# mohakbhardwaj/mjmpc

Hardware: AMD Instinct MI355X
Metric: particle-steps/sec (reacher_7dof-v0 MPPI 4096p x H32 per GPU, control loop incl. noise, rollout, update, shift) (higher is better)
Workload: dtype f64

## Files before the change

### mjmpc_amd/csrc/arm_rollout.hip

```cpp
#include <hip/hip_runtime.h>

#include <cstdlib>
#include <type_traits>

#include "arm_model.h"
#include "arm_rollout.h"
#include "lanegroup.h"
#include "noise_device.h"

namespace mjmpc {
namespace {

template <typename T>
constexpr int newton_maxit() { return sizeof(T) == 4 ? 32 : 12; }

#define PHASE() asm volatile("" ::: "memory")
#define LDS_WAVE_SYNC()                                        \
    do {                                                       \
        __builtin_amdgcn_fence(__ATOMIC_ACQ_REL, "wavefront"); \
        asm volatile("" ::: "memory");                         \
        __builtin_amdgcn_sched_barrier(0);                     \
    } while (0)

constexpr int N_LINK_FIELDS = O_NV / LANES;
__device__ __forceinline__ float uniform_(float x) { return __int_as_float(__builtin_amdgcn_readfirstlane(__float_as_int(x))); }
__device__ __forceinline__ double uniform_(double x) {
    return __hiloint2double(__builtin_amdgcn_readfirstlane(__double2hiint(x)), __builtin_amdgcn_readfirstlane(__double2loint(x)));
}
#ifdef MJMPC_ARM_XJ
constexpr bool XJ = true;
#else
constexpr bool XJ = false;
#endif
template <typename T, bool REG>
struct Model {
    static constexpr bool cached = REG;
    const T* m;
    int l8;
    T reg[REG ? N_LINK_FIELDS : 1];
    T inv_width, mid, inv_mid, inv_omid, dmin, ddiff, solB, solK;
    int ipower;
    __device__ __forceinline__ void cache() {
        if constexpr (REG) {
#pragma unroll
            for (int k = 0; k < N_LINK_FIELDS; ++k) reg[k] = m[k * LANES + l8];
            mid = uniform_(m[O_SOL_MID]);
            inv_width = uniform_(rcp_(m[O_SOL_WIDTH]));
            inv_mid = uniform_(rcp_(mid));
            inv_omid = uniform_(rcp_(T(1) - mid));
            dmin = uniform_(m[O_SOL_DMIN]);
            ddiff = uniform_(m[O_SOL_DMAX] - m[O_SOL_DMIN]);
            solB = uniform_(m[O_SOL_B]);
            solK = uniform_(m[O_SOL_K]);
            ipower = __builtin_amdgcn_readfirstlane((int)m[O_SOL_POWER]);
        }
        cache_xj();
    }
    __device__ __forceinline__ T link(int off, int c = 0) const {
        if constexpr (REG) return reg[off / LANES + c];
        else return m[off + c * LANES + l8];
    }
    __device__ __forceinline__ T glob(int off, int c = 0) const { return m[off + c]; }
    bool xs = false;
    T xf = T(0), xD = T(0), xB = T(0);
    __device__ __forceinline__ void cache_xj() {
        if constexpr (XJ && REG) {
            xs = m[O_JTYPE + l8] != T(0);
            xf = m[O_FLOSS + l8];
            xD = m[O_FLOSS_D + l8];
            xB = uniform_(m[O_FLOSS_B]);
        }
    }
    __device__ __forceinline__ bool xj_slide() const { if constexpr (XJ && REG) return xs; else return XJ && m[O_JTYPE + l8] != T(0); }
    __device__ __forceinline__ T xj_floss() const { if constexpr (XJ && REG) return xf; else return m[O_FLOSS + l8]; }
    __device__ __forceinline__ T xj_floss_D() const { if constexpr (XJ && REG) return xD; else return m[O_FLOSS_D + l8]; }
    __device__ __forceinline__ T xj_floss_B() const { if constexpr (XJ && REG) return xB; else return m[O_FLOSS_B]; }
};

__device__ __forceinline__ float mul_rn(float a, float b) { return __fmul_rn(a, b); }
__device__ __forceinline__ double mul_rn(double a, double b) { return __dmul_rn(a, b); }
__device__ __forceinline__ float add_rn(float a, float b) { return __fadd_rn(a, b); }
__device__ __forceinline__ double add_rn(double a, double b) { return __dadd_rn(a, b); }

template <typename T>
__device__ __forceinline__ void cross(const T* a, const T* b, T* c) {
    c[0] = a[1] * b[2] - a[2] * b[1];
    c[1] = a[2] * b[0] - a[0] * b[2];
    c[2] = a[0] * b[1] - a[1] * b[0];
}
template <typename T>
__device__ __forceinline__ T dot(const T* a, const T* b) { return a[0] * b[0] + a[1] * b[1] + a[2] * b[2]; }
template <typename T>
__device__ __forceinline__ void matvec(const T* R, const T* x, T* y) {
    for (int i = 0; i < 3; ++i) y[i] = R[3 * i] * x[0] + R[3 * i + 1] * x[1] + R[3 * i + 2] * x[2];
}
template <typename T>
__device__ __forceinline__ void symvec(const T* S, const T* x, T* y) {
    y[0] = S[0] * x[0] + S[3] * x[1] + S[4] * x[2];
    y[1] = S[3] * x[0] + S[1] * x[1] + S[5] * x[2];
    y[2] = S[4] * x[0] + S[5] * x[1] + S[2] * x[2];
}

template <int S, typename T>
__device__ __forceinline__ void fk_scan_step(T* R, T* p, int l8) {
    T Ra[9], pa[3], Rn[9], t[3];
    for (int k = 0; k < 9; ++k) Ra[k] = (k % 4 == 0) ? shr<S>(R[k], T(1), l8) : shr0<S>(R[k], l8);
    for (int k = 0; k < 3; ++k) pa[k] = shr0<S>(p[k], l8);
    for (int i = 0; i < 3; ++i)
        for (int j = 0; j < 3; ++j)
            Rn[3 * i + j] = Ra[3 * i] * R[j] + Ra[3 * i + 1] * R[3 + j] + Ra[3 * i + 2] * R[6 + j];
    matvec(Ra, p, t);
    for (int k = 0; k < 3; ++k) p[k] = pa[k] + t[k];
    for (int k = 0; k < 9; ++k) R[k] = Rn[k];
}

template <typename T, typename MT>
__device__ __forceinline__ void row_params(const MT& M, T r, T diag_approx, T jv, T& D, T& aref) {
    if constexpr (MT::cached) {
        T x = fabs(r) * M.inv_width, y;
        x = x > T(1) ? T(1) : x;
        if (M.ipower == 2) {
            T om = T(1) - x;
            y = x <= M.mid ? x * x * M.inv_mid : T(1) - om * om * M.inv_omid;
        } else if (M.ipower == 1) {
            y = x;
        } else {
            const bool lo = x <= M.mid;
            const T xa = lo ? x : T(1) - x, ia = lo ? M.inv_mid : M.inv_omid;
            T qq = xa;
            for (int k = 1; k < M.ipower; ++k) qq *= xa * ia;
            y = lo ? qq : T(1) - qq;
        }
        const T imp = M.dmin + y * M.ddiff;
        T Rr = (T(1) - imp) * rcp_(imp) * diag_approx;
        Rr = Rr < T(1e-15) ? T(1e-15) : Rr;
        D = rcp_(Rr);
        aref = -M.solB * jv - M.solK * imp * r;
        return;
    }
    const T dmin = M.glob(O_SOL_DMIN), dmax = M.glob(O_SOL_DMAX), width = M.glob(O_SOL_WIDTH);
    const T mid = M.glob(O_SOL_MID), power = M.glob(O_SOL_POWER);
    T x = fabs(r) * rcp_(width), y;
    x = x > T(1) ? T(1) : x;
    if (power == T(2)) {
        T om = T(1) - x;
        y = x <= mid ? x * x * rcp_(mid) : T(1) - om * om * rcp_(T(1) - mid);
    } else if (power == T(1)) {
        y = x;
    } else {
        const int n = (int)power;
        const bool lo = x <= mid;
        const T xa = lo ? x : T(1) - x, ma = lo ? mid : T(1) - mid;
        T num = xa, den = T(1);
        for (int k = 1; k < n; ++k) {
            num *= xa;
            den *= ma;
        }
        const T qq = num * rcp_(den);
        y = lo ? qq : T(1) - qq;
    }
    T imp = dmin + y * (dmax - dmin);
    T Rr = (T(1) - imp) * rcp_(imp) * diag_approx;
    Rr = Rr < T(1e-15) ? T(1e-15) : Rr;
    D = rcp_(Rr);
    aref = -M.glob(O_SOL_B) * jv - M.glob(O_SOL_K) * imp * r;
}

template <typename T>
struct Dense {
    T a[21];
    T d[MAX_LINKS];
    static __device__ __forceinline__ constexpr int ix(int i, int j) { return i * (i - 1) / 2 + j; }

    __device__ __forceinline__ void load(const T* tile, const T* diag) {
#pragma unroll
        for (int i = 1; i < MAX_LINKS; ++i)
#pragma unroll
            for (int j = 0; j < i; ++j) a[ix(i, j)] = tile[i * LANES + j];
#pragma unroll
        for (int i = 0; i < MAX_LINKS; ++i) d[i] = diag[i];
    }
    __device__ __forceinline__ void add_rank1(T w, const T* jc) {
#pragma unroll
        for (int i = 0; i < MAX_LINKS; ++i) {
            const T wi = w * jc[i];
            d[i] += wi * jc[i];
#pragma unroll
            for (int j = 0; j < i; ++j) a[ix(i, j)] += wi * jc[j];
        }
    }
    __device__ __forceinline__ void factor() {
#pragma unroll
        for (int k = 0; k < MAX_LINKS; ++k) {
            const T inv = rcp_fast(d[k]);
            d[k] = inv;
#pragma unroll
            for (int i = k + 1; i < MAX_LINKS; ++i) {
                const T aik = a[ix(i, k)];
                const T lik = aik * inv;
#pragma unroll
                for (int j = k + 1; j < i; ++j) a[ix(i, j)] -= aik * a[ix(j, k)];
                d[i] -= aik * lik;
                a[ix(i, k)] = lik;
            }
        }
    }
    __device__ __forceinline__ void solve(T* b) const {
#pragma unroll
        for (int i = 1; i < MAX_LINKS; ++i)
#pragma unroll
            for (int j = 0; j < i; ++j) b[i] -= a[ix(i, j)] * b[j];
#pragma unroll
        for (int i = 0; i < MAX_LINKS; ++i) b[i] *= d[i];
#pragma unroll
        for (int i = MAX_LINKS - 2; i >= 0; --i)
#pragma unroll
            for (int j = i + 1; j < MAX_LINKS; ++j) b[i] -= a[ix(j, i)] * b[j];
    }
};

constexpr int V_DH = LANES * LANES, V_RH = V_DH + LANES, V_DE = V_RH + LANES, V_RE = V_DE + LANES, V_XH = V_RE + LANES,
              V_XE = V_XH + LANES, V_JC = V_XE + LANES, V_TAU = V_JC + LANES, V_EI = V_TAU + LANES,
              PSTRIDE = V_EI + LANES * LANES + 4,
              V_LS = V_XH, V_LD = V_DH, V_LA = V_RH;

template <int K, typename T>
__device__ __forceinline__ void cl_accumulate(const double* __restrict__ W, int A, int nv, int l8, T cq, T cv, double& u) {
    const double qk = (double)bcast<K>(cq), vk = (double)bcast<K>(cv);
    if (K < nv) u += W[K * A + l8] * qk + W[(nv + K) * A + l8] * vk;
    if constexpr (K + 1 < MAX_LINKS) cl_accumulate<K + 1, T>(W, A, nv, l8, cq, cv, u);
}

template <int S, typename T>
__device__ __forceinline__ void mass_diagonals(const T* sw, const T* sv, const T* Fn, const T* Ff, T* d) {
    if constexpr (S == 0) {
        d[0] = dot(sw, Fn) + dot(sv, Ff);
    } else {
        T fn[3], ff[3];
        for (int c = 0; c < 3; ++c) {
            fn[c] = shl_raw<S>(Fn[c]);
            ff[c] = shl_raw<S>(Ff[c]);
        }
        d[S] = dot(sw, fn) + dot(sv, ff);
    }
    if constexpr (S + 1 < MAX_LINKS) mass_diagonals<S + 1, T>(sw, sv, Fn, Ff, d);
}

struct ArmInts {
    int site_link, n_sphere, sph_link, frame_skip, nv;
};

template <typename T>
struct LinkFrame {
    T R[9], p[3], ax[3];
    T mass, a[3], cw[3];
    T Ib[6], hm[3];
    T sw[3], sv[3];
};

template <typename T, typename MT>
__device__ __forceinline__ void kinematics(const MT& M, T sq, T cq, int l8, LinkFrame<T>& L, T q = T(0)) {
    T* R = L.R;
    T* p = L.p;
    T* ax = L.ax;
    const T s = sq, c = cq, tt = T(1) - cq;
    for (int k = 0; k < 3; ++k) { ax[k] = M.link(O_AXIS, k); p[k] = M.link(O_OFF, k); }
    if constexpr (XJ) {
        const T qs = M.xj_slide() ? q : T(0);
        for (int k = 0; k < 3; ++k) p[k] += qs * ax[k];
    }
    R[0] = c + tt * ax[0] * ax[0];
    R[1] = tt * ax[0] * ax[1] - s * ax[2];
    R[2] = tt * ax[0] * ax[2] + s * ax[1];
    R[3] = tt * ax[0] * ax[1] + s * ax[2];
    R[4] = c + tt * ax[1] * ax[1];
    R[5] = tt * ax[1] * ax[2] - s * ax[0];
    R[6] = tt * ax[0] * ax[2] - s * ax[1];
    R[7] = tt * ax[1] * ax[2] + s * ax[0];
    R[8] = c + tt * ax[2] * ax[2];
    fk_scan_step<1>(R, p, l8);
    fk_scan_step<2>(R, p, l8);
    fk_scan_step<4>(R, p, l8);
}

template <typename T, typename MT>
__device__ __forceinline__ void link_frames(const MT& M, LinkFrame<T>& L) {
    const T* R = L.R;
    const T* p = L.p;
    const T mass = L.mass = M.link(O_MASS);
    T t3[3];
    matvec(R, L.ax, L.a);
    {
        const T com[3] = {M.link(O_COM, 0), M.link(O_COM, 1), M.link(O_COM, 2)};
        matvec(R, com, t3);
    }
    T* cw = L.cw;
    for (int k = 0; k < 3; ++k) cw[k] = p[k] + t3[k];
    T* Ib = L.Ib;
    {
        T Il[6], RI[9];
        for (int k = 0; k < 6; ++k) Il[k] = M.link(O_INERTIA, k);
        for (int i = 0; i < 3; ++i) {
            const T* r = R + 3 * i;
            RI[3 * i + 0] = r[0] * Il[0] + r[1] * Il[3] + r[2] * Il[4];
            RI[3 * i + 1] = r[0] * Il[3] + r[1] * Il[1] + r[2] * Il[5];
            RI[3 * i + 2] = r[0] * Il[4] + r[1] * Il[5] + r[2] * Il[2];
        }
        T cc = dot(cw, cw);
        Ib[0] = dot(RI + 0, R + 0) + mass * (cc - cw[0] * cw[0]);
        Ib[1] = dot(RI + 3, R + 3) + mass * (cc - cw[1] * cw[1]);
        Ib[2] = dot(RI + 6, R + 6) + mass * (cc - cw[2] * cw[2]);
        Ib[3] = dot(RI + 0, R + 3) - mass * cw[0] * cw[1];
        Ib[4] = dot(RI + 0, R + 6) - mass * cw[0] * cw[2];
        Ib[5] = dot(RI + 3, R + 6) - mass * cw[1] * cw[2];
    }
    for (int k = 0; k < 3; ++k) { L.hm[k] = mass * cw[k]; L.sw[k] = L.a[k]; }
    cross(p, L.a, L.sv);
    if constexpr (XJ) {
        if (M.xj_slide())
            for (int k = 0; k < 3; ++k) { L.sw[k] = T(0); L.sv[k] = L.a[k]; }
    }
}

template <typename T, typename MT>
__device__ __forceinline__ T bias_force(const MT& M, const LinkFrame<T>& L, T v, int l8) {
    const T *sw = L.sw, *sv = L.sv, *Ib = L.Ib, *hm = L.hm;
    const T mass = L.mass;
    T Vw[3], Vv[3];
    for (int k = 0; k < 3; ++k) {
        Vw[k] = psum(sw[k] * v, l8);
        Vv[k] = psum(sv[k] * v, l8);
    }
    T Aw[3], Av[3];
    {
        T xw[3] = {sw[0] * v, sw[1] * v, sw[2] * v}, xv[3] = {sv[0] * v, sv[1] * v, sv[2] * v};
        T dw[3], d1[3], d2[3];
        cross(Vw, xw, dw);
        cross(Vw, xv, d1);
        cross(Vv, xw, d2);
        for (int k = 0; k < 3; ++k) {
            Aw[k] = psum(dw[k], l8);
            Av[k] = psum(d1[k] + d2[k], l8) - M.glob(O_GRAVITY, k);
        }
    }
    T nV[3], fV[3], nA[3], fA[3], t1[3], t2[3];
    symvec(Ib, Vw, nV);
    cross(hm, Vv, t1);
    cross(hm, Vw, t2);
    for (int k = 0; k < 3; ++k) { nV[k] += t1[k]; fV[k] = mass * Vv[k] - t2[k]; }
    symvec(Ib, Aw, nA);
    cross(hm, Av, t1);
    cross(hm, Aw, t2);
    for (int k = 0; k < 3; ++k) { nA[k] += t1[k]; fA[k] = mass * Av[k] - t2[k]; }
    T c1[3], c2[3], c3[3];
    cross(Vw, nV, c1);
    cross(Vv, fV, c2);
    cross(Vw, fV, c3);
    T fn[3], ff[3];
    for (int k = 0; k < 3; ++k) {
        fn[k] = ssum(nA[k] + c1[k] + c2[k], l8);
        ff[k] = ssum(fA[k] + c3[k], l8);
    }
    return dot(sw, fn) + dot(sv, ff);
}

template <typename T>
__device__ __forceinline__ T mass_matrix_tile(const LinkFrame<T>& L, int l8, T* ldsM) {
    const T *sw = L.sw, *sv = L.sv;
    T d[MAX_LINKS];
    {
        T mc = ssum(L.mass, l8), hc[3], Ic[6];
        for (int k = 0; k < 3; ++k) hc[k] = ssum(L.hm[k], l8);
        for (int k = 0; k < 6; ++k) Ic[k] = ssum(L.Ib[k], l8);
        T Fn[3], Ff[3], t1[3], t2[3];
        symvec(Ic, sw, Fn);
        cross(hc, sv, t1);
        cross(hc, sw, t2);
        for (int k = 0; k < 3; ++k) { Fn[k] += t1[k]; Ff[k] = mc * sv[k] - t2[k]; }
        mass_diagonals<0, T>(sw, sv, Fn, Ff, d);
    }
#pragma unroll
    for (int sft = 0; sft < MAX_LINKS; ++sft) {
        if (l8 + sft < MAX_LINKS) {
            ldsM[l8 * LANES + l8 + sft] = d[sft];
            ldsM[(l8 + sft) * LANES + l8] = d[sft];
        }
    }
    return d[0];
}

template <int S0, int S1, typename T>
__device__ __forceinline__ T mass_matrix_tile_part(const LinkFrame<T>& L, int l8, T* ldsM) {
    const T *sw = L.sw, *sv = L.sv;
    T d[MAX_LINKS];
#pragma unroll
    for (int k = 0; k < MAX_LINKS; ++k) d[k] = T(0);
    T mc = ssum(L.mass, l8), hc[3], Ic[6];
    for (int k = 0; k < 3; ++k) hc[k] = ssum(L.hm[k], l8);
    for (int k = 0; k < 6; ++k) Ic[k] = ssum(L.Ib[k], l8);
    T Fn[3], Ff[3], t1[3], t2[3];
    symvec(Ic, sw, Fn);
    cross(hc, sv, t1);
    cross(hc, sw, t2);
    for (int k = 0; k < 3; ++k) { Fn[k] += t1[k]; Ff[k] = mc * sv[k] - t2[k]; }
    auto diag_s = [&](auto SC) {
        constexpr int S = decltype(SC)::value;
        if constexpr (S >= S0 && S < S1) {
            if constexpr (S == 0) {
                d[0] = dot(sw, Fn) + dot(sv, Ff);
            } else {
                T fn[3], ff[3];
                for (int c = 0; c < 3; ++c) { fn[c] = shl_raw<S>(Fn[c]); ff[c] = shl_raw<S>(Ff[c]); }
                d[S] = dot(sw, fn) + dot(sv, ff);
            }
        }
    };
    diag_s(std::integral_constant<int, 0>()); diag_s(std::integral_constant<int, 1>()); diag_s(std::integral_constant<int, 2>());
    diag_s(std::integral_constant<int, 3>()); diag_s(std::integral_constant<int, 4>()); diag_s(std::integral_constant<int, 5>());
    diag_s(std::integral_constant<int, 6>());
#pragma unroll
    for (int sft = S0; sft < S1; ++sft) {
        if (l8 + sft < MAX_LINKS) {
            ldsM[l8 * LANES + l8 + sft] = d[sft];
            ldsM[(l8 + sft) * LANES + l8] = d[sft];
        }
    }
    return d[0];
}

template <typename T, typename MT>
__device__ __forceinline__ void contact_geometry(const MT& M, const ArmInts& I, const LinkFrame<T>& L,
                                                 const T* ctr, T v, int l8, T& cdist, bool& cinst, T& jc, T& jv) {
    const T pn[3] = {M.glob(O_PLANE_N, 0), M.glob(O_PLANE_N, 1), M.glob(O_PLANE_N, 2)};
    const T sph_r = M.glob(O_SPH_R);
    cdist = dot(ctr, pn) - M.glob(O_PLANE_D) - sph_r;
    cinst = cdist < M.glob(O_SPH_MARGIN);
    jc = T(0);
    jv = T(0);
    if (__any(cinst)) {
        T r[3], ar[3];
        for (int k = 0; k < 3; ++k) r[k] = ctr[k] - pn[k] * (sph_r + T(0.5) * cdist) - L.p[k];
        cross(L.a, r, ar);
        T jl = dot(pn, ar);
        if constexpr (XJ) jl = M.xj_slide() ? dot(pn, L.a) : jl;
        jc = (cinst && l8 <= I.sph_link) ? jl : T(0);
        jv = gsum(jc * v);
    }
}

enum Role : int { SOLO = 0, DYN = 1, SOLVE = 2,
                  QDYN = 3, QSOLVE = 4, QMASS = 5, QAUX = 6 };
template <int ROLE>
__device__ __forceinline__ constexpr int role_slot() {
    return (ROLE == SOLVE || ROLE == QSOLVE) ? 1 : (ROLE == QMASS ? 2 : (ROLE == QAUX ? 3 : 0));
}
template <int ROLE>
__device__ __forceinline__ constexpr bool role_counts() { return ROLE == SOLO || ROLE == DYN || ROLE == QDYN; }

struct Stamps {
#if defined(MJMPC_STAMPS) && defined(MJMPC_STAMPS_ABS)
    long long acc[16];
    int nsub;
    __device__ __forceinline__ void begin() { for (int k = 0; k < 16; ++k) acc[k] = 0; nsub = 0; }
    __device__ __forceinline__ void mark(int k) {
        if (nsub == MJMPC_STAMPS_ABS) acc[k] = clock64();
        if (k == 13 || k == 15) ++nsub;
    }
    __device__ __forceinline__ void flush(unsigned* diag, int wave, int lane) {
        if (diag && blockIdx.x == 0 && lane == 0)
            for (int k = 0; k < 16; ++k) ((unsigned long long*)diag)[2 + 16 * wave + k] = (unsigned long long)acc[k];
    }
#elif defined(MJMPC_STAMPS)
    long long last, acc[16];
    __device__ __forceinline__ void begin() { for (int k = 0; k < 16; ++k) acc[k] = 0; last = clock64(); }
#ifdef MJMPC_STAMPS_MASK
    __device__ __forceinline__ void mark(int k) {
        if (!((MJMPC_STAMPS_MASK >> k) & 1)) return;
        const long long t = clock64(); acc[k] += t - last; last = t;
    }
#else
#ifdef MJMPC_STAMPS_FENCE
    __device__ __forceinline__ void mark(int k) {
        __builtin_amdgcn_sched_barrier(0);
        const long long t = clock64(); acc[k] += t - last; last = t;
        __builtin_amdgcn_sched_barrier(0);
    }
#else
    __device__ __forceinline__ void mark(int k) { const long long t = clock64(); acc[k] += t - last; last = t; }
#endif
#endif
    __device__ __forceinline__ void flush(unsigned* diag, int wave, int lane) {
        if (diag && blockIdx.x == 0 && lane == 0)
            for (int k = 0; k < 16; ++k) ((unsigned long long*)diag)[2 + 16 * wave + k] = (unsigned long long)acc[k];
    }
#else
    __device__ __forceinline__ void begin() {}
    __device__ __forceinline__ void mark(int) {}
    __device__ __forceinline__ void flush(unsigned*, int, int) {}
#endif
};

__device__ __forceinline__ void duo_barrier() {
    asm volatile("s_waitcnt lgkmcnt(0)\n\ts_barrier" ::: "memory");
    __builtin_amdgcn_sched_barrier(0);
}

template <typename T>
struct FlossRow {
    T f = T(0), D = T(0), aref = T(0);
    int z = 0;
    __device__ __forceinline__ int zone_at(T xa) const {
        if (!(f > T(0))) return 0;
        const T sl = D * (xa - aref);
        const T bc = sizeof(T) == 4 ? T(2e-5) * (fabs(sl) + f) : T(0);
        if (z < 0) return sl > -f + bc ? (sl >= f ? 1 : 0) : -1;
        if (z > 0) return sl < f - bc ? (sl <= -f ? -1 : 0) : 1;
        return sl <= -f - bc ? -1 : (sl >= f + bc ? 1 : 0);
    }
    __device__ __forceinline__ T diag() const { return (f > T(0) && z == 0) ? D : T(0); }
    __device__ __forceinline__ T rhs() const { return f > T(0) ? (z == 0 ? D * aref : (z < 0 ? f : -f)) : T(0); }
    __device__ __forceinline__ T force(T xa) const { return f > T(0) ? (z == 0 ? -D * (xa - aref) : (z < 0 ? f : -f)) : T(0); }
    __device__ __forceinline__ int memory() const { return f > T(0) ? (16 | ((z + 1) << 5)) : 0; }
};
template <typename T, typename MT>
__device__ __forceinline__ FlossRow<T> floss_row(const MT& M, T v, int rows) {
    FlossRow<T> r;
    if constexpr (XJ) {
        r.f = M.xj_floss();
        if (r.f > T(0)) {
            r.D = M.xj_floss_D();
            r.aref = -M.xj_floss_B() * v;
            r.z = (rows & 16) ? ((rows >> 5) & 3) - 1 : 0;
        }
    }
    return r;
}

template <typename T, typename MT>
__device__ __forceinline__ T xj_line_search(const MT& M, T* ldsM, int l8, T a_prev, T a_new, T tau, T sig, T D, T aref,
                                            bool inst, T jc, T Dc, T arefc, bool cinst, const FlossRow<T>& fl) {
    const T d = a_new - a_prev;
    ldsM[V_XH + l8] = a_prev;
    ldsM[V_XE + l8] = d;
    LDS_WAVE_SYNC();
    T Ma = M.link(O_ARMATURE) * a_prev, Md = M.link(O_ARMATURE) * d;
#pragma unroll
    for (int j = 0; j < MAX_LINKS; ++j) {
        const T m = ldsM[l8 * LANES + j];
        Ma += m * ldsM[V_XH + j];
        Md += m * ldsM[V_XE + j];
    }
    const T g0 = gsum(d * (Ma - tau)), h0 = gsum(d * Md);
    const T rl0 = sig * a_prev - aref, rld = sig * d;
    const T rf0 = a_prev - fl.aref, rfd = d;
    T rc0 = T(0), rcd = T(0);
    const bool any_c = __any(cinst);
    if (any_c) { rc0 = gsum(jc * a_prev) - arefc; rcd = gsum(jc * d); }
    T alpha = T(1);
    T lo = T(0), hi = T(0);
    bool have_hi = false;
#pragma unroll 1
    for (int k = 0; k < 12; ++k) {
        T g = T(0), hh = T(0);
        if (inst) { const T r = rl0 + alpha * rld; if (r < T(0)) { g += D * r * rld; hh += D * rld * rld; } }
        if (fl.f > T(0)) {
            const T sl = fl.D * (rf0 + alpha * rfd);
            if (sl <= -fl.f) g -= fl.f * rfd;
            else if (sl >= fl.f) g += fl.f * rfd;
            else { g += sl * rfd; hh += fl.D * rfd * rfd; }
        }
        T gp = gsum(g), hp = gsum(hh);
        if (cinst) { const T r = rc0 + alpha * rcd; if (r < T(0)) { gp += Dc * r * rcd; hp += Dc * rcd * rcd; } }
        const T dphi = g0 + alpha * h0 + gp, ddphi = h0 + hp;
        const bool pos = dphi > T(0);
        if (pos) { hi = alpha; have_hi = true; } else lo = alpha;
        const T tol = T(sizeof(T) == 4 ? 1e-6 : 1e-14) * (fabs(g0) + fabs(h0) + T(1e-30));
        const bool done = fabs(dphi) <= tol || !(ddphi > T(0));
        T next = alpha - dphi * rcp_(ddphi > T(0) ? ddphi : T(1));
        if (have_hi && !(next > lo && next < hi)) next = T(0.5) * (lo + hi);
        if (!have_hi && !(next > lo)) next = T(2) * alpha + T(1);
        if (!done) alpha = next;
        if (!__any(!done)) break;
    }
    return a_prev + alpha * d;
}

template <typename T>
__device__ __forceinline__ void active_set(T aw, T sig, T aref, T jc, T arefc, bool inst, bool cinst, bool act,
                                           bool cact, bool& act2, bool& cact2) {
    if constexpr (sizeof(T) == 4) {
        const T res = sig * aw - aref, resc = gsum(jc * aw) - arefc;
        const T band = T(4e-6) * (fabs(aref) + fabs(aw) + T(1));
        const T bandc = T(4e-6) * (fabs(arefc) + fabs(resc + arefc) + T(1));
        act2 = inst && (act ? !(res > band) : (res < -band));
        cact2 = cinst && (cact ? !(resc > bandc) : (resc < -bandc));
    } else {
        act2 = inst && (sig * aw - aref < T(0));
        cact2 = cinst && (gsum(jc * aw) - arefc < T(0));
    }
}

template <typename T>
__device__ __forceinline__ constexpr bool rows_by_dyn() { return sizeof(T) == 8; }

template <typename T, typename MT>
__device__ __forceinline__ void limit_row(const MT& M, T q, T v, T& sig, T& D, T& aref) {
    T dist = T(0);
    sig = T(0);
    if (M.link(O_LIMITED) != T(0)) {
        const T dlo = q - M.link(O_RANGE_LO), dhi = M.link(O_RANGE_HI) - q;
        if (dlo < T(0)) { sig = T(1); dist = dlo; }
        else if (dhi < T(0)) { sig = T(-1); dist = dhi; }
    }
    D = T(0);
    aref = T(0);
    if (__any(sig != T(0))) {
        row_params(M, dist, M.link(O_DOF_INVW), sig * v, D, aref);
        D = sig != T(0) ? D : T(0);
        aref = sig != T(0) ? aref : T(0);
    }
}

constexpr int RST_EVER = 8, RST_REAL = 16, RST_INF = 32, RST_OPTS = RST_REAL | RST_INF;
struct ResetCtl {
    bool any = false;
    bool count = false;
};
template <int ROLE, typename T>
__device__ __forceinline__ int rflags(const T* ldsM) { return (int)ldsM[PSTRIDE - 4 + role_slot<ROLE>()]; }
template <int ROLE, typename T>
__device__ __forceinline__ void rflags_set(T* ldsM, int f) { ldsM[PSTRIDE - 4 + role_slot<ROLE>()] = (T)f; }
struct NoResetRecord {
    __device__ __forceinline__ const double* operator()() const { return nullptr; }
};
__device__ __forceinline__ unsigned long long particle_lanes(int lane) { return 0x5555ull << ((lane & 0x30) | (lane & 1)); }
template <typename T>
__device__ __forceinline__ bool mj_is_bad(T x) { return !(fabs(x) <= T(1e10)); }
template <int ROLE, typename T>
__device__ __forceinline__ void reset_check_start(ResetCtl& rc, T q, T v, int lane, T* ldsM) {
    const unsigned long long bal = __ballot(mj_is_bad(q) || mj_is_bad(v));
    if (bal != 0ull) {
        rc.any = true;
        if (bal & particle_lanes(lane)) rflags_set<ROLE>(ldsM, rflags<ROLE>(ldsM) | 2);
    }
}

template <int ROLE, typename T, typename MT>
__device__ __forceinline__ void arm_front(const MT& M, const ArmInts& I, T& q, T& v, T& aw, T& sq, T& cq,
                                          int& rows, T tau_act, T* ldsM, int lane, int l8, T* site,
                                          unsigned* diag, bool& free_step, Stamps& ST, ResetCtl* rc = nullptr) {
    free_step = false;
#ifdef MJMPC_NO_RESET
    rc = nullptr;
#endif
    if (rc && __builtin_expect(rc->any, 0)) {
        int f = rflags<ROLE>(ldsM) & ~4;
        if (f & 2) {
            q = T(0); v = T(0); sq = T(0); cq = T(1); aw = T(0);
            rows = 0;
            f = (f & RST_OPTS) | 1 | RST_EVER;
            if (role_counts<ROLE>() && diag && l8 == 0 && rc->count) { atomicAdd(diag + 1, 1u); if (f & RST_REAL) atomicAdd(diag + 2, 1u); }
        }
        rflags_set<ROLE>(ldsM, f);
        if (f & 1) tau_act = M.link(O_GEAR) * fmin(fmax(T(0), M.link(O_CTRL_LO)), M.link(O_CTRL_HI));
    }
    PHASE();
    LinkFrame<T> L;
    kinematics(M, sq, cq, l8, L, q);
    if constexpr (ROLE != SOLVE) {
        const T sp[3] = {M.glob(O_SITE_POS, 0), M.glob(O_SITE_POS, 1), M.glob(O_SITE_POS, 2)};
        T t[3];
        matvec(L.R, sp, t);
        for (int k = 0; k < 3; ++k) site[k] = L.p[k] + t[k];
    }
    T ctr[3] = {T(0), T(0), T(0)};
    bool near_plane = false;
    if (ROLE != DYN && I.n_sphere > 0) {
        const T sp[3] = {M.glob(O_SPH_POS, 0), M.glob(O_SPH_POS, 1), M.glob(O_SPH_POS, 2)};
        T t[3];
        matvec(L.R, sp, t);
        for (int k = 0; k < 3; ++k) t[k] += L.p[k];
        if constexpr (ROLE == SOLVE) {
            const T pn[3] = {M.glob(O_PLANE_N, 0), M.glob(O_PLANE_N, 1), M.glob(O_PLANE_N, 2)};
            const bool mine = dot(t, pn) - M.glob(O_PLANE_D) - M.glob(O_SPH_R) < M.glob(O_SPH_MARGIN);
            const unsigned long long bal = __ballot(mine);
            near_plane = (bal >> lane_of_link(lane, I.sph_link)) & 1ull;
            if (__any(near_plane))
                for (int k = 0; k < 3; ++k) ctr[k] = __shfl(t[k], lane_of_link(lane, I.sph_link));
        } else {
            for (int k = 0; k < 3; ++k) ctr[k] = __shfl(t[k], lane_of_link(lane, I.sph_link));
        }
    }
    ST.mark(0);
    PHASE();
    link_frames(M, L);
    ST.mark(1);

    if constexpr (ROLE == DYN) {
        const T bias = bias_force(M, L, v, l8);
        ldsM[V_TAU + l8] = -bias - M.link(O_DAMPING) * v + tau_act;
        if constexpr (rows_by_dyn<T>()) {
            T sg, Dl, al;
            limit_row(M, q, v, sg, Dl, al);
            ldsM[V_LS + l8] = sg;
            ldsM[V_LD + l8] = Dl;
            ldsM[V_LA + l8] = al;
        }
        ST.mark(2);
        duo_barrier();
        ST.mark(3);
        Dense<T> F;
        F.load(ldsM, ldsM + V_DE);
        F.factor();
        T col[MAX_LINKS];
#pragma unroll
        for (int i = 0; i < MAX_LINKS; ++i) col[i] = (i == l8) ? T(1) : T(0);
        F.solve(col);
#pragma unroll
        for (int i = 0; i < MAX_LINKS; ++i) ldsM[V_EI + l8 * LANES + i] = col[i];
        ST.mark(6);
        duo_barrier();
        ST.mark(7);
        return;
    }

    T bias = T(0);
    if constexpr (ROLE == SOLO) bias = bias_force(M, L, v, l8);
    T dgM = T(0);
    const T damping = M.link(O_DAMPING), h = M.glob(O_TIMESTEP);
    dgM = mass_matrix_tile(L, l8, ldsM);
    dgM += M.link(O_ARMATURE);
    ldsM[V_DE + l8] = dgM + h * damping;
    if constexpr (ROLE == SOLO) LDS_WAVE_SYNC();
    ST.mark(4);

    T tau = -bias - damping * v + tau_act;
    if constexpr (ROLE == SOLVE) {
        duo_barrier();
        ST.mark(3);
        tau = ldsM[V_TAU + l8];
    }
    T ei[MAX_LINKS];

    T sig = T(0), dist = T(0), D = T(0), aref = T(0);
    bool inst = false;
    constexpr bool rows_from_dyn = ROLE == SOLVE && rows_by_dyn<T>();
    if constexpr (rows_from_dyn) {
        sig = ldsM[V_LS + l8];
        D = ldsM[V_LD + l8];
        aref = ldsM[V_LA + l8];
        inst = sig != T(0);
    } else if (M.link(O_LIMITED) != T(0)) {
        T dlo = q - M.link(O_RANGE_LO), dhi = M.link(O_RANGE_HI) - q;
        if (dlo < T(0)) { sig = T(1); dist = dlo; inst = true; }
        else if (dhi < T(0)) { sig = T(-1); dist = dhi; inst = true; }
    }
    bool cinst = false;
    T jc = T(0), Dc = T(0), arefc = T(0);
    if (I.n_sphere > 0 && (ROLE != SOLVE || __any(near_plane))) {
        T cdist, jv;
        contact_geometry(M, I, L, ctr, v, l8, cdist, cinst, jc, jv);
        if constexpr (ROLE == SOLVE) {
            cinst = cinst && near_plane;
            jc = near_plane ? jc : T(0);
        }
        if (__any(cinst)) {
            row_params(M, cdist - M.glob(O_SPH_MARGIN), M.glob(O_SPH_INVW), jv, Dc, arefc);
            Dc = cinst ? Dc : T(0);
            arefc = cinst ? arefc : T(0);
        }
    }
    FlossRow<T> fl = floss_row(M, v, rows);
    const bool any_rows = __any(inst || cinst || (XJ && fl.f > T(0)));
    if (!any_rows) rows = 0;
    if constexpr (!rows_from_dyn) {
        if (any_rows) {
            row_params(M, dist, M.link(O_DOF_INVW), sig * v, D, aref);
            D = inst ? D : T(0);
            aref = inst ? aref : T(0);
        }
    }
    ST.mark(5);
    bool act = inst && ((rows & 1) ? (rows & 2) != 0 : true);
    bool cact = cinst && ((rows & 4) ? (rows & 8) != 0 : true);
    bool changed = false;
    const bool any_c = __any(cinst);
    T qfrc_c = T(0);

    if constexpr (ROLE == SOLVE) {
        if (any_rows) {
            if (any_c) ldsM[V_JC + l8] = jc;
            changed = true;
            for (int it = 0; it < newton_maxit<T>(); ++it) {
                T rhs = tau + (act ? D * sig * aref : T(0));
                if (any_c) rhs += cact ? Dc * jc * arefc : T(0);
                T dh = dgM + (act ? D : T(0));
                if constexpr (XJ) { rhs += fl.rhs(); dh += fl.diag(); }
                ldsM[V_DH + l8] = dh;
                ldsM[V_RH + l8] = rhs;
                LDS_WAVE_SYNC();
                Dense<T> F;
                F.load(ldsM, ldsM + V_DH);
                T rh[MAX_LINKS];
#pragma unroll
                for (int i = 0; i < MAX_LINKS; ++i) rh[i] = ldsM[V_RH + i];
                if (any_c && __any(cact)) {
                    T jv[MAX_LINKS];
#pragma unroll
                    for (int i = 0; i < MAX_LINKS; ++i) jv[i] = ldsM[V_JC + i];
                    F.add_rank1(cact ? Dc : T(0), jv);
                }
                F.factor();
                T col[MAX_LINKS];
#pragma unroll
                for (int i = 0; i < MAX_LINKS; ++i) col[i] = (i == l8) ? T(1) : T(0);
                F.solve(col);
                ST.mark(it == 0 ? 6 : 9);
                if (it == 0 && !rows_by_dyn<T>()) {
                    duo_barrier();
#pragma unroll
                    for (int i = 0; i < MAX_LINKS; ++i) ei[i] = ldsM[V_EI + l8 * LANES + i];
                }
                T acc = T(0);
#pragma unroll
                for (int i = 0; i < MAX_LINKS; ++i) acc += col[i] * rh[i];
                if constexpr (XJ) {
                    if (it > 0) acc = xj_line_search(M, ldsM, l8, aw, acc, tau, sig, D, aref, inst, jc, Dc, arefc, cinst, fl);
                }
                aw = acc;
                bool act2, cact2;
                active_set(aw, sig, aref, jc, arefc, inst, cinst, act, cact, act2, cact2);
                bool flip = act2 != act, cflip = cact2 != cact;
                changed = flip || cflip;
                act = act2;
                cact = cact2;
                bool fflip = false;
                if constexpr (XJ) {
                    const int z2 = fl.zone_at(aw);
                    fflip = z2 != fl.z;
                    fl.z = z2;
                    changed = changed || fflip;
                }
                if (it == 0 && rows_by_dyn<T>()) {
                    duo_barrier();
#pragma unroll
                    for (int i = 0; i < MAX_LINKS; ++i) ei[i] = ldsM[V_EI + l8 * LANES + i];
                }
                ST.mark(it == 0 ? 8 : 9);
                if (!__any(changed)) break;
                const float nflip = gsum(flip ? 1.0f : 0.0f);
                if (!XJ && !__any(cflip || nflip > 1.5f || fflip)) {
                    if (flip) {
                        T zjj = col[0];
#pragma unroll
                        for (int i = 1; i < MAX_LINKS; ++i) zjj = (l8 == i) ? col[i] : zjj;
                        const T c = act ? D : -D;
                        ldsM[V_XH + 0] = (T)l8;
                        ldsM[V_XH + 1] = c;
                        ldsM[V_XH + 2] = c * sig * aref;
                        ldsM[V_XH + 3] = zjj;
                        ldsM[V_XH + 4] = aw;
                    }
                    LDS_WAVE_SYNC();
                    if (nflip > 0.5f) {
                        const int j = (int)ldsM[V_XH + 0];
                        const T c = ldsM[V_XH + 1], dl = ldsM[V_XH + 2], zjj = ldsM[V_XH + 3], aj = ldsM[V_XH + 4];
                        T z = col[0];
#pragma unroll
                        for (int i = 1; i < MAX_LINKS; ++i) z = (j == i) ? col[i] : z;
                        const T yj = aj + dl * zjj;
                        aw = (aw + dl * z) - c * z * yj * rcp_(T(1) + c * zjj);
                    }
                    active_set(aw, sig, aref, jc, arefc, inst, cinst, act, cact, act2, cact2);
                    changed = (act2 != act) || (cact2 != cact);
                    act = act2;
                    cact = cact2;
                    if constexpr (XJ) {
                        const int z2 = fl.zone_at(aw);
                        changed = changed || z2 != fl.z;
                        fl.z = z2;
                    }
                    ST.mark(9);
                    if (!__any(changed)) break;
                }
                LDS_WAVE_SYNC();
            }
            if (changed && diag) atomicAdd(diag, 1u);
            rows = (inst ? 1 : 0) | (act ? 2 : 0) | (cinst ? 4 : 0) | (cact ? 8 : 0) | fl.memory();
            qfrc_c = act ? -D * (sig * aw - aref) * sig : T(0);
            if constexpr (XJ) qfrc_c += fl.force(aw);
            if (__any(cact)) {
                T fcn = cact ? -Dc * (gsum(jc * aw) - arefc) : T(0);
                qfrc_c += jc * fcn;
            }
        }
        ldsM[V_RE + l8] = tau + qfrc_c;
        if (!any_rows) {
            duo_barrier();
#pragma unroll
            for (int i = 0; i < MAX_LINKS; ++i) ei[i] = ldsM[V_EI + l8 * LANES + i];
        } else {
            LDS_WAVE_SYNC();
        }
        ST.mark(7);
        T x = T(0);
#pragma unroll
        for (int i = 0; i < MAX_LINKS; ++i) x += ei[i] * ldsM[V_RE + i];
        ldsM[V_XE + l8] = x;
        free_step = !any_rows;
        ST.mark(10);
        return;
    }

    const bool roleH = l8 < 4;
    Dense<T> F;
    if (any_rows) {
        changed = true;
        if (any_c) ldsM[V_JC + l8] = jc;
        for (int it = 0; it < newton_maxit<T>(); ++it) {
            T rhs = tau + (act ? D * sig * aref : T(0));
            if (any_c) rhs += cact ? Dc * jc * arefc : T(0);
            T dh = dgM + (act ? D : T(0));
            if constexpr (XJ) { rhs += fl.rhs(); dh += fl.diag(); }
            ldsM[V_DH + l8] = dh;
            ldsM[V_RH + l8] = rhs;
            LDS_WAVE_SYNC();
            if (it == 0 || roleH) {
                F.load(ldsM, ldsM + (roleH ? V_DH : V_DE));
                if (any_c && __any(cact)) {
                    T jv[MAX_LINKS];
#pragma unroll
                    for (int i = 0; i < MAX_LINKS; ++i) jv[i] = ldsM[V_JC + i];
                    F.add_rank1((roleH && cact) ? Dc : T(0), jv);
                }
                F.factor();
            }
            ST.mark(it == 0 ? 6 : 9);
            if (roleH) {
                T b[MAX_LINKS];
#pragma unroll
                for (int i = 0; i < MAX_LINKS; ++i) b[i] = ldsM[V_RH + i];
                F.solve(b);
#pragma unroll
                for (int i = 0; i < MAX_LINKS; ++i) ldsM[V_XH + i] = b[i];
            }
            LDS_WAVE_SYNC();
            if constexpr (XJ) {
                const T a_new = ldsM[V_XH + l8];
                LDS_WAVE_SYNC();
                aw = it > 0 ? xj_line_search(M, ldsM, l8, aw, a_new, tau, sig, D, aref, inst, jc, Dc, arefc, cinst, fl) : a_new;
            } else {
                aw = ldsM[V_XH + l8];
            }
            bool act2, cact2;
            active_set(aw, sig, aref, jc, arefc, inst, cinst, act, cact, act2, cact2);
            changed = (act2 != act) || (cact2 != cact);
            act = act2;
            cact = cact2;
            if constexpr (XJ) {
                const int z2 = fl.zone_at(aw);
                changed = changed || z2 != fl.z;
                fl.z = z2;
            }
            ST.mark(it == 0 ? 8 : 9);
            if (!__any(changed)) break;
        }
        if (changed && diag) atomicAdd(diag, 1u);
        rows = (inst ? 1 : 0) | (act ? 2 : 0) | (cinst ? 4 : 0) | (cact ? 8 : 0) | fl.memory();
        qfrc_c = act ? -D * (sig * aw - aref) * sig : T(0);
        if constexpr (XJ) qfrc_c += fl.force(aw);
        if (__any(cact)) {
            T fcn = cact ? -Dc * (gsum(jc * aw) - arefc) : T(0);
            qfrc_c += jc * fcn;
        }
        ldsM[V_RE + l8] = tau + qfrc_c;
        LDS_WAVE_SYNC();
    } else {
        ldsM[V_RE + l8] = tau;
        LDS_WAVE_SYNC();
        F.load(ldsM, ldsM + V_DE);
        F.factor();
    }
    if (!roleH) {
        T b[MAX_LINKS];
#pragma unroll
        for (int i = 0; i < MAX_LINKS; ++i) b[i] = ldsM[V_RE + i];
        F.solve(b);
#pragma unroll
        for (int i = 0; i < MAX_LINKS; ++i) ldsM[V_XE + i] = b[i];
    }
    free_step = !any_rows;
    ST.mark(10);
}

typedef __attribute__((address_space(3))) int* qflag_ptr;
__device__ __forceinline__ int q_read(qflag_ptr qf, int which) {
// ... 333 lines not shown
    }
    ST.mark(12);
    const T h = M.glob(O_TIMESTEP);
    if (free_step) aw = x;
    v = add_rn(v, mul_rn(h, x));
    const T dq = mul_rn(h, v);
    q = add_rn(q, dq);
    const bool slide = M.xj_slide();
    const T dqa = slide ? T(0) : dq;
    T sd, cd;
    const bool big = __any(!(fabs(dq) <= (slide ? T(1e5) : T(0.25))));
    if (__builtin_expect(big, 0)) {
        sincos_small(dqa * T(1.0 / 256.0), sd, cd);
        for (int k = 0; k < 8; ++k) {
            const T s2 = T(2) * sd * cd;
            cd = T(1) - T(2) * sd * sd;
            sd = s2;
        }
    } else {
        sincos_small(dqa, sd, cd);
    }
    const T s1 = sq * cd + cq * sd, c1 = cq * cd - sq * sd;
    const T k = T(1.5) - T(0.5) * (s1 * s1 + c1 * c1);
    sq = s1 * k;
    cq = c1 * k;
#ifdef MJMPC_NO_RESET
    rc = nullptr;
#endif
    if (rc && __builtin_expect(big, 0)) {
        const unsigned long long bal = __ballot(mj_is_bad(x) || mj_is_bad(q) || mj_is_bad(v));
        if (bal != 0ull) {
            rc->any = true;
            const unsigned long long mine = particle_lanes(lane);
            const double* rst = record();
            if (rst == nullptr) {
            } else if (__ballot(mj_is_bad(x)) & mine) {
                q = (T)rst[l8];
                v = (T)rst[LANES + l8];
                sq = (T)rst[2 * LANES + 3 + l8];
                cq = (T)rst[3 * LANES + 3 + l8];
                aw = T(0);
                const int f0 = rflags<ROLE>(ldsM);
                rflags_set<ROLE>(ldsM, f0 | 1 | 4 | RST_EVER);
                if (role_counts<ROLE>() && diag && l8 == 0 && rc->count) { atomicAdd(diag + 1, 1u); if (f0 & RST_REAL) atomicAdd(diag + 2, 1u); }
            } else if (bal & mine) {
                rflags_set<ROLE>(ldsM, rflags<ROLE>(ldsM) | 2);
            }
        }
    }
    LDS_WAVE_SYNC();
    ST.mark(13);
}

constexpr int MONO_RED = 32;

template <typename T, bool DUO, typename MT>
__device__ __forceinline__ void real_env_step(const MT& M, const ArmInts& I, const MonoStep& mo, double* st, T q, T v,
                                              const T* tgt, const double* action, int A, T* lds, int lane, int wave, int l8,
                                              int g, unsigned* diag) {
    const int nv = I.nv;
    T* ldsM = lds + g * PSTRIDE;
    T aw = T(0);
    if (l8 >= nv) { q = T(0); v = T(0); }
    T sinq, cosq;
    sincos_(q, sinq, cosq);
    if constexpr (XJ) { if (M.xj_slide()) { sinq = T(0); cosq = T(1); } }
    int rows = 0;
    Stamps ST;
    ST.begin();
    bool fs = false;
    ResetCtl rc;
    rc.count = g == 0;
    if (DUO && wave == 1) rflags_set<SOLVE>(ldsM, RST_REAL);
    else rflags_set<SOLO>(ldsM, RST_REAL);
    auto record = [&mo]() -> const double* { return mo.reset_rec; };
    if (mo.reset_rec) {
        if (DUO && wave == 1) reset_check_start<SOLVE>(rc, q, v, lane, ldsM);
        else reset_check_start<SOLO>(rc, q, v, lane, ldsM);
    }
    if (DUO && wave == 1) {
        if constexpr (DUO) {
            T nosite[3];
            for (int sub = 0; sub < I.frame_skip; ++sub) {
                arm_front<SOLVE>(M, I, q, v, aw, sinq, cosq, rows, T(0), ldsM, lane, l8, nosite, diag, fs, ST, &rc);
                arm_back<SOLVE>(M, q, v, aw, sinq, cosq, ldsM, l8, fs, ST, lane, &rc, nullptr, record);
            }
        }
        return;
    }
    constexpr int R = DUO ? DYN : SOLO;
    const T u = l8 < A ? (T)action[l8] : T(0);
    const T tau_act = M.link(O_GEAR) * fmin(fmax(u, M.link(O_CTRL_LO)), M.link(O_CTRL_HI));
    T site[3];
    unsigned* dcount = diag;
    for (int sub = 0; sub < I.frame_skip; ++sub) {
        if (R == DYN && sub > 0) arm_back<R>(M, q, v, aw, sinq, cosq, ldsM, l8, fs, ST, lane, &rc, dcount, record);
        arm_front<R>(M, I, q, v, aw, sinq, cosq, rows, tau_act, ldsM, lane, l8, site, dcount, fs, ST, &rc);
        if constexpr (R == SOLO) arm_back<R>(M, q, v, aw, sinq, cosq, ldsM, l8, fs, ST, lane, &rc, dcount, record);
    }
    const int site_lane = lane_of_link(lane, I.site_link);
    for (int k = 0; k < 3; ++k) site[k] = __shfl(site[k], site_lane);
    if constexpr (R == DYN) arm_back<R>(M, q, v, aw, sinq, cosq, ldsM, l8, fs, ST, lane, &rc, dcount, record);
    if (rc.any && (rflags<R>(ldsM) & 4))
        for (int k = 0; k < 3; ++k) site[k] = (T)mo.reset_rec[2 * LANES + k];
    if (g == 0) {
        const T dx = site[0] - tgt[0], dy = site[1] - tgt[1], dz = site[2] - tgt[2];
        if (mo.step_cost && l8 == 0)
            ((T*)mo.step_cost)[0] = fabs(dx) + fabs(dy) + fabs(dz) + T(5) * sqrt_(dx * dx + dy * dy + dz * dz);
        if (mo.step_nobs) {
            T* o = (T*)mo.step_nobs;
            if (l8 < nv) { o[l8] = q; o[nv + l8] = v; }
            if (l8 < 3) {
                const T hh = l8 == 0 ? site[0] : (l8 == 1 ? site[1] : site[2]);
                const T gg = l8 == 0 ? tgt[0] : (l8 == 1 ? tgt[1] : tgt[2]);
                o[2 * nv + l8] = hh;
                o[2 * nv + 3 + l8] = hh - gg;
            }
        }
        if (l8 < nv) {
            st[l8] = (double)q;
            st[LANES + l8] = (double)v;
        }
    }
}

template <typename T, int NT>
__device__ __forceinline__ void mono_record(double lam, double* __restrict__ rec_out, int HA, double* red, const T* actT) {
    const int tid = threadIdx.x;
    __syncthreads();
    if (tid < LANES) {
        const double q = red[tid], x = q == INFINITY ? -INFINITY : (-1.0 / lam) * q;
        double m = x;
        for (int o = 1; o < LANES; o <<= 1) m = fmax(m, __shfl_xor(m, o));
        const double e = x == -INFINITY ? 0.0 : exp(x - m);
        double S = e;
        for (int o = 1; o < LANES; o <<= 1) S += __shfl_xor(S, o);
        red[LANES + tid] = e;
        if (tid == 0) { rec_out[0] = m; rec_out[1] = S; }
    }
    __syncthreads();
    double e[LANES];
#pragma unroll
    for (int k = 0; k < LANES; ++k) e[k] = red[LANES + k];
    for (int j = tid; j < HA; j += NT) {
        double acc = 0.0;
#pragma unroll
        for (int k = 0; k < LANES; ++k) acc += e[k] * (double)actT[k * HA + j];
        rec_out[2 + j] = acc;
    }
}

constexpr int MAX_A = 8;
constexpr int FIN_CHUNK = 4;
template <typename T>
__global__ __launch_bounds__(128) void arm_mppi_finish_kernel(const T* __restrict__ model, const double* __restrict__ recs, long n_rec,
                                                              int H, int A, const double* __restrict__ mean_in,
                                                              double* __restrict__ mean_out, const MonoStep mo,
                                                              int env_step, unsigned* diag) {
    __shared__ __attribute__((aligned(16))) T lds[LANES * PSTRIDE + ARM_BLOB_LEN + 3];
    __shared__ double sh[2 * (2 + MAX_A)];
    const int tid = threadIdx.x, t = blockIdx.x, HA = H * A, rec = 2 + HA;
    const int lane = tid & 63, wave = __builtin_amdgcn_readfirstlane(tid >> 6);
    const bool stepper = t == 0 && env_step && mo.state_io && !mo.record;
    double rm[FIN_CHUNK], rs[FIN_CHUNK], rw[FIN_CHUNK][MAX_A];
    auto fetch = [&](long base) {
#pragma unroll
        for (int k = 0; k < FIN_CHUNK; ++k) {
            const long b = base + tid + 128L * k;
            const double* r = recs + (b < n_rec ? b : 0) * rec;
            rm[k] = b < n_rec ? r[0] : -INFINITY;
            rs[k] = r[1];
#pragma unroll
            for (int a = 0; a < MAX_A; ++a) rw[k][a] = a < A ? r[2 + t * A + a] : 0.0;
        }
    };
    fetch(0);
    const double mean_old = (tid < A && !mo.record) ? mean_in[t * A + tid] : 0.0;
    const long long count = (t == 0 && mo.step_counter) ? *mo.step_counter : 0;
    const int l8 = lane_link(lane), g = lane_slot(lane);
    T q0 = T(0), v0 = T(0), tgt[3] = {T(0), T(0), T(0)};
    if (stepper) {
        for (int k = tid; k < ARM_BLOB_LEN; k += 128) lds[LANES * PSTRIDE + k] = model[k];
        for (int k = tid; k < LANES * PSTRIDE; k += 128) lds[k] = T(0);
        q0 = (T)mo.state_io[l8];
        v0 = (T)mo.state_io[LANES + l8];
        for (int k = 0; k < 3; ++k) tgt[k] = (T)mo.state_io[2 * LANES + k];
    }
    double m = -INFINITY, S = 0.0, W[MAX_A];
#pragma unroll
    for (int a = 0; a < MAX_A; ++a) W[a] = 0.0;
    for (long base = 0; base < n_rec; base += 128L * FIN_CHUNK) {
        if (base > 0) fetch(base);
        double mn = m;
#pragma unroll
        for (int k = 0; k < FIN_CHUNK; ++k) mn = fmax(mn, rm[k]);
        const double sc = m == -INFINITY ? 0.0 : exp(m - mn);
        S *= sc;
#pragma unroll
        for (int a = 0; a < MAX_A; ++a) W[a] *= sc;
#pragma unroll
        for (int k = 0; k < FIN_CHUNK; ++k) {
            const double c = rm[k] == -INFINITY ? 0.0 : exp(rm[k] - mn);
            S += c * rs[k];
#pragma unroll
            for (int a = 0; a < MAX_A; ++a) W[a] += c * rw[k][a];
        }
        m = mn;
    }
    double M = m;
    for (int o = 32; o > 0; o >>= 1) M = fmax(M, __shfl_xor(M, o));
    if (lane == 0) sh[wave] = M;
    __syncthreads();
    M = fmax(sh[0], sh[1]);
    const double f = m == -INFINITY ? 0.0 : exp(m - M);
    S *= f;
    for (int o = 32; o > 0; o >>= 1) S += __shfl_xor(S, o);
#pragma unroll
    for (int a = 0; a < MAX_A; ++a) {
        W[a] *= f;
        for (int o = 32; o > 0; o >>= 1) W[a] += __shfl_xor(W[a], o);
    }
    __syncthreads();
    if (lane == 0) {
        sh[wave * (2 + MAX_A) + 1] = S;
#pragma unroll
        for (int a = 0; a < MAX_A; ++a) sh[wave * (2 + MAX_A) + 2 + a] = W[a];
    }
    __syncthreads();
    S = sh[1] + sh[(2 + MAX_A) + 1];
    const double wsum = tid < A ? sh[2 + tid] + sh[(2 + MAX_A) + 2 + tid] : 0.0;
    if (mo.record) {
        if (tid < A) mo.record[2 + t * A + tid] = wsum;
        if (t == 0 && tid == 0) { mo.record[0] = M; mo.record[1] = S; }
        return;
    }
    double nm = 0.0;
    if (tid < A) {
        nm = (1.0 - mo.step_size) * mean_old + mo.step_size * (wsum / S);
        if (mo.shift_mode < 0) {
            mean_out[t * A + tid] = nm;
        } else {
            if (t > 0) mean_out[(t - 1) * A + tid] = nm;
            if (t == H - 1) mean_out[t * A + tid] = mo.shift_mode == 0 ? 0.0 : nm;
        }
    }
    if (t != 0) return;
    __syncthreads();
    if (tid < A) sh[tid] = nm;
    double* slot = mo.action_host ? mo.action_host + (count & 1) * (A + 1) : nullptr;
    if (tid < A) {
        if (mo.action_out) mo.action_out[tid] = nm;
        if (slot) __hip_atomic_store(slot + tid, nm, __ATOMIC_RELAXED, __HIP_MEMORY_SCOPE_SYSTEM);
    }
    if (wave == 0) {
        asm volatile("s_waitcnt vmcnt(0)" ::: "memory");
        if (tid == 0) {
            if (mo.step_counter) *mo.step_counter = count + 1;
            if (slot) __hip_atomic_store(slot + A, (double)(count + 1), __ATOMIC_RELAXED, __HIP_MEMORY_SCOPE_SYSTEM);
        }
    }
    if (!stepper) return;
    __syncthreads();
    Model<T, true> Mv{lds + LANES * PSTRIDE, l8};
    Mv.cache();
    ArmInts I;
    I.site_link = (int)lds[LANES * PSTRIDE + O_SITE_LINK];
    I.n_sphere = (int)lds[LANES * PSTRIDE + O_N_SPHERE];
    I.sph_link = (int)lds[LANES * PSTRIDE + O_SPH_LINK];
    I.frame_skip = (int)lds[LANES * PSTRIDE + O_FRAME_SKIP];
    I.nv = (int)lds[LANES * PSTRIDE + O_NV];
    I.site_link = __builtin_amdgcn_readfirstlane(I.site_link);
    I.n_sphere = __builtin_amdgcn_readfirstlane(I.n_sphere);
    I.sph_link = __builtin_amdgcn_readfirstlane(I.sph_link);
    I.frame_skip = __builtin_amdgcn_readfirstlane(I.frame_skip);
    I.nv = __builtin_amdgcn_readfirstlane(I.nv);
    real_env_step<T, true>(Mv, I, mo, mo.state_io, q0, v0, tgt, sh, A, lds, lane, wave, l8, g, diag);
}


template <typename T, bool STEP, bool CL, int WAVES, bool DUO, bool MONO>
__global__ __launch_bounds__(DUO ? 128 : 64) __attribute__((amdgpu_waves_per_eu(WAVES, WAVES))) void arm_rollout_kernel(const T* __restrict__ model, const double* state,
                                                         long P, int H, int A, const double* mean,
                                                         const T* __restrict__ noise, T* __restrict__ cost,
                                                         T* __restrict__ act, T* __restrict__ obs,
                                                         T* __restrict__ nobs, double* state_out, unsigned* diag,
                                                         RolloutFusion fuse, const MonoStep mono_arg) {
    const MonoStep* mop = &mono_arg;
    constexpr int SHAPE = DUO ? 2 : 1, NW = SHAPE;
    constexpr bool QUAD = false;
    const qflag_ptr qf = nullptr;
    int seq = 0;
#include "arm_rollout_body.inc"
}
template <typename T, int NW, bool MONO>
__global__ __launch_bounds__(64 * NW) __attribute__((amdgpu_waves_per_eu(1, 1))) void arm_rollout_flags_kernel(const T* __restrict__ model, const double* state,
                                                         long P, int H, int A, const double* mean,
                                                         const T* __restrict__ noise, T* __restrict__ cost,
                                                         T* __restrict__ act, T* __restrict__ obs,
                                                         T* __restrict__ nobs, unsigned* diag,
                                                         RolloutFusion fuse, const MonoStep mono_arg) {
    const MonoStep* mop = &mono_arg;
    constexpr int SHAPE = 10 + NW;
    constexpr bool STEP = false, CL = false, DUO = false, QUAD = true;
    double* const state_out = nullptr;
    __shared__ int qflags[QF_COUNT];
    qflag_ptr qf = (qflag_ptr)qflags;
    int seq = 0;
#include "arm_rollout_body.inc"
// ... 99 lines not shown
```

Baseline: 660.8 million.

## Store mass tile as upper rows only and move limit rows to solver

The mass-matrix tile is now written once per lane as a contiguous row with stride LANES+1 (diagonal-shifted), instead of writing both symmetric halves. Readers (Dense::load and the line search) are changed to index the transposed/upper half to match. Joint-limit row computation moves from the DYN role to the SOLVE role before the first barrier, dropping LDS traffic for those values, and the finish kernel gets a waves-per-EU attribute under the XJ build. Indexing consistency between the new stride and the readers is the main risk.

Result: faster. 681.7 million, median of 6 (+3.2%).

```diff
diff --git a/mjmpc_amd/csrc/arm_rollout.hip b/mjmpc_amd/csrc/arm_rollout.hip
--- a/mjmpc_amd/csrc/arm_rollout.hip
+++ b/mjmpc_amd/csrc/arm_rollout.hip
@@ -176,7 +176,7 @@
 #pragma unroll
         for (int i = 1; i < MAX_LINKS; ++i)
 #pragma unroll
-            for (int j = 0; j < i; ++j) a[ix(i, j)] = tile[i * LANES + j];
+            for (int j = 0; j < i; ++j) a[ix(i, j)] = tile[j * LANES + i];
 #pragma unroll
         for (int i = 0; i < MAX_LINKS; ++i) d[i] = diag[i];
     }
@@ -244,6 +244,16 @@
         d[S] = dot(sw, fn) + dot(sv, ff);
     }
     if constexpr (S + 1 < MAX_LINKS) mass_diagonals<S + 1, T>(sw, sv, Fn, Ff, d);
+}
+
+template <int S0, int S1, typename T>
+__device__ __forceinline__ void tile_store(const T* d, int l8, T* ldsM) {
+    static_assert(S0 >= 0 && S1 <= MAX_LINKS, "d[] holds the diagonals 0 ... MAX_LINKS - 1");
+    T* row = ldsM + l8 * (LANES + 1);
+    if (l8 < MAX_LINKS) {
+#pragma unroll
+        for (int sft = S0; sft < S1; ++sft) row[sft] = d[sft];
+    }
 }
 
 struct ArmInts {
@@ -379,13 +389,7 @@
         for (int k = 0; k < 3; ++k) { Fn[k] += t1[k]; Ff[k] = mc * sv[k] - t2[k]; }
         mass_diagonals<0, T>(sw, sv, Fn, Ff, d);
     }
-#pragma unroll
-    for (int sft = 0; sft < MAX_LINKS; ++sft) {
-        if (l8 + sft < MAX_LINKS) {
-            ldsM[l8 * LANES + l8 + sft] = d[sft];
-            ldsM[(l8 + sft) * LANES + l8] = d[sft];
-        }
-    }
+    tile_store<0, MAX_LINKS>(d, l8, ldsM);
     return d[0];
 }
 
@@ -418,13 +422,7 @@
     diag_s(std::integral_constant<int, 0>()); diag_s(std::integral_constant<int, 1>()); diag_s(std::integral_constant<int, 2>());
     diag_s(std::integral_constant<int, 3>()); diag_s(std::integral_constant<int, 4>()); diag_s(std::integral_constant<int, 5>());
     diag_s(std::integral_constant<int, 6>());
-#pragma unroll
-    for (int sft = S0; sft < S1; ++sft) {
-        if (l8 + sft < MAX_LINKS) {
-            ldsM[l8 * LANES + l8 + sft] = d[sft];
-            ldsM[(l8 + sft) * LANES + l8] = d[sft];
-        }
-    }
+    tile_store<S0, S1>(d, l8, ldsM);
     return d[0];
 }
 
@@ -546,7 +544,7 @@
     T Ma = M.link(O_ARMATURE) * a_prev, Md = M.link(O_ARMATURE) * d;
 #pragma unroll
     for (int j = 0; j < MAX_LINKS; ++j) {
-        const T m = ldsM[l8 * LANES + j];
+        const T m = ldsM[j < l8 ? j * LANES + l8 : l8 * LANES + j];
         Ma += m * ldsM[V_XH + j];
         Md += m * ldsM[V_XE + j];
     }
@@ -601,7 +599,7 @@
 }
 
 template <typename T>
-__device__ __forceinline__ constexpr bool rows_by_dyn() { return sizeof(T) == 8; }
+__device__ __forceinline__ constexpr bool rows_before_e1() { return sizeof(T) == 8; }
 
 template <typename T, typename MT>
 __device__ __forceinline__ void limit_row(const MT& M, T q, T v, T& sig, T& D, T& aref) {
@@ -699,13 +697,6 @@
     if constexpr (ROLE == DYN) {
         const T bias = bias_force(M, L, v, l8);
         ldsM[V_TAU + l8] = -bias - M.link(O_DAMPING) * v + tau_act;
-        if constexpr (rows_by_dyn<T>()) {
-            T sg, Dl, al;
-            limit_row(M, q, v, sg, Dl, al);
-            ldsM[V_LS + l8] = sg;
-            ldsM[V_LD + l8] = Dl;
-            ldsM[V_LA + l8] = al;
-        }
         ST.mark(2);
         duo_barrier();
         ST.mark(3);
@@ -734,6 +725,15 @@
     if constexpr (ROLE == SOLO) LDS_WAVE_SYNC();
     ST.mark(4);
 
+    T sig = T(0), dist = T(0), D = T(0), aref = T(0);
+    bool inst = false;
+    constexpr bool rows_early = ROLE == SOLVE && rows_before_e1<T>();
+    if constexpr (rows_early) {
+        limit_row(M, q, v, sig, D, aref);
+        inst = sig != T(0);
+        ST.mark(2);
+    }
+
     T tau = -bias - damping * v + tau_act;
     if constexpr (ROLE == SOLVE) {
         duo_barrier();
@@ -742,18 +742,12 @@
     }
     T ei[MAX_LINKS];
 
-    T sig = T(0), dist = T(0), D = T(0), aref = T(0);
-    bool inst = false;
-    constexpr bool rows_from_dyn = ROLE == SOLVE && rows_by_dyn<T>();
-    if constexpr (rows_from_dyn) {
-        sig = ldsM[V_LS + l8];
-        D = ldsM[V_LD + l8];
-        aref = ldsM[V_LA + l8];
-        inst = sig != T(0);
-    } else if (M.link(O_LIMITED) != T(0)) {
-        T dlo = q - M.link(O_RANGE_LO), dhi = M.link(O_RANGE_HI) - q;
-        if (dlo < T(0)) { sig = T(1); dist = dlo; inst = true; }
-        else if (dhi < T(0)) { sig = T(-1); dist = dhi; inst = true; }
+    if constexpr (!rows_early) {
+        if (M.link(O_LIMITED) != T(0)) {
+            T dlo = q - M.link(O_RANGE_LO), dhi = M.link(O_RANGE_HI) - q;
+            if (dlo < T(0)) { sig = T(1); dist = dlo; inst = true; }
+            else if (dhi < T(0)) { sig = T(-1); dist = dhi; inst = true; }
+        }
     }
     bool cinst = false;
     T jc = T(0), Dc = T(0), arefc = T(0);
@@ -773,7 +767,7 @@
     FlossRow<T> fl = floss_row(M, v, rows);
     const bool any_rows = __any(inst || cinst || (XJ && fl.f > T(0)));
     if (!any_rows) rows = 0;
-    if constexpr (!rows_from_dyn) {
+    if constexpr (!rows_early) {
         if (any_rows) {
             row_params(M, dist, M.link(O_DOF_INVW), sig * v, D, aref);
             D = inst ? D : T(0);
@@ -816,7 +810,7 @@
                 for (int i = 0; i < MAX_LINKS; ++i) col[i] = (i == l8) ? T(1) : T(0);
                 F.solve(col);
                 ST.mark(it == 0 ? 6 : 9);
-                if (it == 0 && !rows_by_dyn<T>()) {
+                if (it == 0 && !rows_before_e1<T>()) {
                     duo_barrier();
 #pragma unroll
                     for (int i = 0; i < MAX_LINKS; ++i) ei[i] = ldsM[V_EI + l8 * LANES + i];
@@ -841,7 +835,7 @@
                     fl.z = z2;
                     changed = changed || fflip;
                 }
-                if (it == 0 && rows_by_dyn<T>()) {
+                if (it == 0 && rows_before_e1<T>()) {
                     duo_barrier();
 #pragma unroll
                     for (int i = 0; i < MAX_LINKS; ++i) ei[i] = ldsM[V_EI + l8 * LANES + i];
@@ -1481,8 +1475,13 @@
 
 constexpr int MAX_A = 8;
 constexpr int FIN_CHUNK = 4;
+#ifdef MJMPC_ARM_XJ
+#define MJMPC_FINISH_WAVES __attribute__((amdgpu_waves_per_eu(1, 1)))
+#else
+#define MJMPC_FINISH_WAVES
+#endif
 template <typename T>
-__global__ __launch_bounds__(128) void arm_mppi_finish_kernel(const T* __restrict__ model, const double* __restrict__ recs, long n_rec,
+__global__ __launch_bounds__(128) MJMPC_FINISH_WAVES void arm_mppi_finish_kernel(const T* __restrict__ model, const double* __restrict__ recs, long n_rec,
                                                               int H, int A, const double* __restrict__ mean_in,
                                                               double* __restrict__ mean_out, const MonoStep mo,
                                                               int env_step, unsigned* diag) {
```
